# TF2-Engine/TF2

Hardware: AMD Instinct MI355X
Metric: images/sec ResNet50 INT4w/INT8a (higher is better)
Workload: dtype int8

## Files before the change

### tf2_amd/csrc/net.hip

```cpp
#include <hip/hip_runtime.h>
#include <algorithm>
#include <cstdio>
#include <cstdlib>
#include <cstring>
#include <map>
#include <mutex>
#include "tf2_net.h"
#include "tf2_device.h"
#include "opts.h"

namespace tf2 {

static thread_local std::string g_err;
void set_error(const std::string& s) { g_err = s; }
const std::string& last_error() { return g_err; }

#define HIP_OK(expr)                                                                   \
  do {                                                                                 \
    hipError_t e_ = (expr);                                                            \
    if (e_ != hipSuccess) {                                                            \
      set_error(std::string(#expr) + ": " + hipGetErrorString(e_));                    \
      return TF2_ERR_HIP;                                                              \
    }                                                                                  \
  } while (0)
// ... 280 lines not shown
  wp.scratch_bytes = (wp.scratch_bytes + 255) / 256 * 256;
  if (wp.ks_ctr_bytes) {
    wp.ks_part_off = wp.scratch_off + wp.scratch_bytes;
    wp.ks_part_bytes = (size_t)std::max(1, opts.sk_kb_blocks) * std::max(1, opts.sk_kb_max) * 16384;
    wp.scratch_bytes += wp.ks_part_bytes;
  }
  wp.total_bytes = wp.scratch_off + wp.scratch_bytes;
  auto res = plans.emplace(key, std::move(wp));
  return &res.first->second;
}

void Net::load_options() {
  RunOpts o;
  o.flags |= (int)opt("exp", 0) & 0x7ff8;
  o.pw_mode = (int)opt("pw", o.pw_mode);
  o.sk_mode = (int)opt("sk", o.sk_mode);
  o.sk8_blocks = (long)opt("sk8", o.sk8_blocks);
  o.bg_poll_limit = (long)opt("bgroup_polls", o.bg_poll_limit); o.bg_withhold = (long)opt("bgroup_withhold", 0);
  o.sk_s3_blocks = (long)opt("sk_s3", o.sk_s3_blocks); o.sk_s3_blocks_conc = (long)opt("sk_s3_conc", o.sk_s3_blocks_conc);
  o.fc_mode = (int)opt("fc", o.fc_mode);
  o.fc_min_slabs = (int)opt("fc_min", o.fc_min_slabs);
  o.c3_mode = (int)opt("c3", o.c3_mode);
  o.c3_min_blocks = (long)opt("c3_min", o.c3_min_blocks);
  o.c3_min256 = (long)opt("c3_min256", o.c3_min256);
  o.c3_w9 = (int)opt("c3_w9", o.c3_w9);
  o.c3_pool = (int)opt("c3_pool", o.c3_pool);
  o.first_fuse = (int)opt("first", o.first_fuse);
  o.first_pool = (int)opt("first_pool", o.first_pool);
  o.fire_mode = (int)opt("fire", o.fire_mode);
  o.fire_pool = (int)opt("fire_pool", o.fire_pool);
  o.bneck_min_blocks = (long)opt("bneck_min", o.bneck_min_blocks);
  o.stem_mode = (int)opt("stem", o.stem_mode);
  o.bgroup_min7 = (int)opt("bgroup_min7", o.bgroup_min7);
  o.bgroup_min14 = (int)opt("bgroup_min14", o.bgroup_min14);
  o.bgroup_min28 = (int)opt("bgroup_min28", o.bgroup_min28);
  o.bgroup_min56f = (int)opt("bgroup_min56f", o.bgroup_min56f);
  o.bgroup_chain = (int)opt("bgroup_chain", o.bgroup_chain);
  o.bgroup_mode = (int)opt("bgroup", o.bgroup_mode);
  o.bfirst_mode = (int)opt("bfirst", o.bfirst_mode);
  o.bfirst_min = (int)opt("bfirst_min", o.bfirst_min);
  o.bband_mode = (int)opt("bband", o.bband_mode);
  o.bband_rows = (int)opt("bband_rows", o.bband_rows);
  o.bband_rows_alone = (int)opt("bband_rows_alone", o.bband_rows_alone);
  o.bband_rows_dd = (int)opt("bband_rows_dd", o.bband_rows_dd);
  o.c3_min_hw = (int)opt("c3_min_hw", o.c3_min_hw);
  o.bband_min = (int)opt("bband_min", o.bband_min);
// ... 53 lines not shown
      if (st.sel == Launch::SEL_FIRST) { FirstArgs f = st.first; f.p = pa; return f.pool ? launch_conv_first_pool(f, stream) : launch_conv_first(f, stream); }
      return launch_prep_input(pa, stream);
    }
    case Launch::POOL: return launch_maxpool(st.pool, stream);
    case Launch::AVG: return launch_global_avg(st.avg, stream);
    case Launch::L2N: return launch_l2norm(st.l2n, stream);
    case Launch::CONV:
      switch (st.sel) {
        case Launch::SEL_PW: return launch_conv_pw(st.conv, st.TM, stream);
        case Launch::SEL_PWK: return launch_conv_pwk(st.conv, st.TM, stream);
        case Launch::SEL_PWKPAIR: return launch_conv_pwk_pair(st.conv, st.TM, st.conv2, st.TM2, stream);
        case Launch::SEL_SK:
          if (logits && lp->logits_direct >= 0 && &st == &lp->steps[lp->logits_direct]) {
            ConvArgs cd = st.conv_direct; cd.y = logits;
            return launch_conv_mfma_sk(cd, opts.sk8_blocks, st.shape, stream);
          }
          return launch_conv_mfma_sk(st.conv, opts.sk8_blocks, st.shape, stream);
        case Launch::SEL_MFMA2: return launch_conv_mfma2(st.conv, st.TM, stream);
        case Launch::SEL_BNECK: return launch_conv_bneck(st.bneck, st.TM, st.shape, stream);
        case Launch::SEL_PAIR: return launch_conv_mfma2_pair(st.conv, st.conv2, st.TM, stream);
        case Launch::SEL_SKPAIR: return launch_conv_mfma_sk_pair(st.conv, st.conv2, opts.sk8_blocks, st.shape, stream);
        case Launch::SEL_BBAND: return launch_conv_bband(st.bband, st.bg_c, st.bg_m, stream);
        case Launch::SEL_C3: return launch_conv_c3(st.c3, stream);
        case Launch::SEL_FIRE: return launch_conv_fire(st.fire, stream);
        case Launch::SEL_FC: return launch_conv_fc(st.fc, stream);
        case Launch::SEL_BGROUPF: return launch_conv_bgroup_first(st.bgroup, stream);
        case Launch::SEL_BFIRST: return launch_conv_bfirst(st.bgroup, stream);
        case Launch::SEL_BGROUP:
          if (!st.bg_chain.empty()) return launch_conv_bgroup(st.bg_chain.data(), (int)st.bg_chain.size(), st.bg_hw, st.bg_c, st.bg_m, stream);
          return launch_conv_bgroup(&st.bgroup, 1, st.bg_hw, st.bg_c, st.bg_m, stream);
        case Launch::SEL_STEM: return launch_conv_stem(st.stem, st.shape, stream);
        default: return launch_conv_shift(st.conv, st.signed_in, st.mul24, st.shape, stream);
      }
  }
  return -1;
}

tf2_status Net::describe_launches(int batch, bool concurrent, std::vector<std::pair<int, LaunchRecord>>* out) {
  std::lock_guard<std::mutex> lock(run_mutex);
  if (!packed_valid) { set_error("tf2_net_describe_launches: no packed image"); return TF2_ERR_STATE; }
  if (batch <= 0) { set_error("tf2_net_describe_launches: batch must be positive"); return TF2_ERR_ARG; }
  const WorkPlan* wp = plan(batch, false);
  const uint8_t* saved = packed_dev;
  if (!packed_dev) packed_dev = packed.data();
  static char fake_ws[16];
  std::list<LaunchPlan> keep;
// ... 246 lines not shown
```

### tf2_amd/csrc/net_plan.hip

```cpp
#include <hip/hip_runtime.h>
#include <algorithm>
#include <map>
#include <mutex>
#include <string>
#include <vector>
#include "tf2_net.h"
#include "tf2_device.h"

namespace tf2 {

bool Net::pair_candidate(int l) const {
  if (l < 1 || l + 1 >= nd.n_layers) return false;
  const tf2_layer_desc& A = layers[l]; const tf2_layer_desc& B = layers[l + 1];
  for (const tf2_layer_desc* L : {&A, &B})
    if (L->ipool || L->pool_en || L->endpool || L->concat >= 0 || L->src < 0) return false;
  if (B.src == l || B.add_src == l) return false;
  if (A.add_src >= 0 || B.add_src >= 0) return false;
  const PackLayer* pa = pack_layer(l); const PackLayer* pb = pack_layer(l + 1);
  if (!pa || !pb || pa->kind != KIND_MFMA || pb->kind != KIND_MFMA) return false;
  if (pa->fuse_next > 0 || pa->fused_into >= 0 || pb->fuse_next > 0 || pb->fused_into >= 0) return false;
  return true;
}

bool Net::bgroup_first_at(int l) const {
// ... 112 lines not shown
  if (L.ipool || L.k != 3 || L.stride != 1 || L.dil != 1 || L.pad_h != 1 || L.pad_w != 1 || L.src < 0 || L.add_src >= 0 || L.endpool) return false;
  if (layers[L.src].concat >= 0 || out_Cp[L.src] != L.C || L.OH != L.H || L.OW != L.W) return false;
  const PackLayer* pl = pack_layer(l);
  if (!pl || pl->kind != KIND_MFMA || (pl->TM != 64 && pl->TM != 128) || pl->w_share || pl->signed_in) return false;
  if (pl->Cp_in != L.C || pl->Cp_in % 64 != 0 || pl->nslab != 9 * (pl->Cp_in / 64) || (long)pl->n_entries != (long)pl->n_mtiles * pl->nslab) return false;
  if (pl->fuse_next > 0 || pl->fused_into >= 0) return false;
  const bool one_window = pl->n_phases == 1 && !pl->dual, dual = pl->n_phases == 2 && pl->dual;
  if (!one_window && !dual) return false;
  return conv_c3_shape_ok(L.H, L.W, L.C, pl->Np, opts.c3_min_hw);
}

bool Net::fc_at(int l, int batch) const {
  const tf2_layer_desc& L = layers[l];
  if (l == nd.n_layers - 1) return false;
  { const PackLayer* p4 = pack_layer(l); if (batch > 32 && !(p4 && p4->fc4)) return false; }
  if (L.ipool || L.k != L.H || L.k != L.W || L.stride != 1 || L.dil != 1 || L.pad_h || L.pad_w || L.OH != 1 || L.OW != 1) return false;
  if (L.src < 0 || L.add_src >= 0 || L.endpool || L.pool_en || L.concat >= 0 || layers[L.src].concat >= 0 || out_Cp[L.src] != L.C) return false;
  const PackLayer* pl = pack_layer(l);
  if (!pl || pl->kind != KIND_MFMA || (pl->TM != 64 && pl->TM != 128) || pl->w_share || pl->signed_in || pl->Np % 128 != 0) return false;
  if (pl->Cp_in != L.C || pl->Cp_in % 64 != 0 || pl->nslab != L.k * L.k * (pl->Cp_in / 64) || (long)pl->n_entries != (long)pl->n_mtiles * pl->nslab) return false;
  if ((pl->nslab < opts.fc_min_slabs && !pl->fc4) || pl->fuse_next > 0 || pl->fused_into >= 0) return false;
  const bool one_window = pl->n_phases == 1 && !pl->dual, dual = pl->n_phases == 2 && pl->dual;
  return one_window || dual;
}

bool Net::stem_selected(int batch) const {
  const tf2_layer_desc& L0 = layers[0];
  const PackLayer* p0 = pack_layer(0);
  const long long pixels = (long long)batch * L0.H * L0.W;
  return opts.stem_mode != 0 && p0 && p0->kind == KIND_MFMA && p0->off_w2 != 0 && nd.conv1_rewrite && nd.image_c == 3 &&
         in_layout[0].Cp_in == 64 && in_layout[0].half == 32 && L0.OH == L0.H - 2 && L0.OW == L0.W - 2 &&
         pixels * 64 < (1ll << 31) && (long long)batch * 3 * nd.image_h * nd.image_w < (1ll << 31);
}

static bool device_fits_group_launches() {
  int dev = 0;
  if (hipGetDevice(&dev) != hipSuccess) return true;
  static std::mutex mu;
  static std::map<int, int> n_cu;
  std::lock_guard<std::mutex> lock(mu);
  auto it = n_cu.find(dev);
  if (it == n_cu.end()) {
    hipDeviceProp_t prop;
    const int n = hipGetDeviceProperties(&prop, dev) == hipSuccess ? prop.multiProcessorCount : 256;
    it = n_cu.emplace(dev, n).first;
  }
// ... 385 lines not shown
    if (opts.c3_mode == 2) tmk = 64; else if (opts.c3_mode == 3 && pm->Np % 128 == 0) tmk = 128;
    Launch sc;
    if (!((long)batch * tiles * (pm->Np / tmk) >= opts.c3_min_blocks && conv_step(l, sc, false) && pm->TM == sc.TM)) return false;
    const ConvArgs& c = sc.conv;
    C3Args& f = sc.c3;
    f.x = c.x; f.y = c.y; f.w = c.w; f.hdr = c.hdr; f.hdr_bytes = c.hdr_bytes; f.zero2 = c.zero; f.tm = sc.TM; f.tmk = tmk;
    f.dbg = dbg_ptr(l);
    f.B = batch; f.H = L.H; f.W = L.W; f.C = L.C; f.M = pm->Np; f.x_cp = c.g.Cp_in;
    f.TH = th; f.TW = tw; f.tiles_x = tiles_x; f.tiles_per_img = tiles;
    set_fast_div((uint32_t)tw, &f.tw_m, &f.tw_s); set_fast_div((uint32_t)(tw + 2), &f.hc_m, &f.hc_s);
    set_fast_div((uint32_t)tiles_x, &f.tx_m, &f.tx_s); set_fast_div((uint32_t)tiles, &f.tpi_m, &f.tpi_s);
    f.relu = c.g.relu; f.fast = c.g.fast; f.dbl = c.g.dbl_out; f.dual = c.dual;
    f.y_cp = c.g.y_cp; f.y_off = c.g.y_off; f.y_nvalid = c.g.y_nvalid;
    if (pool_in) {
      const TensorPlan& to = T(E.out_tensor);
      f.pool = 1; f.PH = L.PH; f.PW = L.PW; f.y = base + to.offset; f.y_cp = to.Cp; f.y_off = E.out_off;
    }
    f.w9 = conv_c3_takes_w9(f, opts.c3_w9) ? 1 : 0;
    sc.sel = Launch::SEL_C3;
    st = sc;
    return pool_in;
  }

  bool bneck_fuse(int l, const tf2_layer_desc& L, const PackLayer* pl, Launch& st) {
    fused_done[pl->fuse_next] = 1;
    Launch sb;
    if (!conv_step(pl->fuse_next, sb, false)) return false;
    const PackLayer* pb = n.pack_layer(pl->fuse_next);
    BneckArgs& f = st.bneck;
    const ConvArgs& ca = st.conv; const ConvArgs& cb = sb.conv;
    f.x = ca.x; f.y_mid = ca.y; f.ymid_cp = ca.g.y_cp;
    f.w1 = ca.w; f.hdr1 = ca.hdr; f.hdr1_used = round_up((5 + pl->n_phases) * pl->TM * 4, 1024);
    f.dual1 = pl->dual; f.fast1 = pl->fast; f.relu1 = ca.g.relu;
    f.w2 = cb.w; f.hdr2 = cb.hdr; f.hdr2_bytes = cb.hdr_bytes; f.hdr2_used = round_up((5 + pb->n_phases) * pb->TM * 4, 1024);
    f.dual2 = pb->dual; f.fast2 = pb->fast; f.relu2 = cb.g.relu;
    f.y = cb.y; f.y_cp = cb.g.y_cp; f.y_off = cb.g.y_off; f.y_nvalid = cb.g.y_nvalid;
    f.res = cb.res; f.res_cp = cb.g.res_cp; f.res_off = cb.g.res_off; f.add_relu = cb.g.add_relu; f.has_res = cb.g.has_res;
    f.zero = ca.zero; f.keep_mid = wp->keep_all ? 1 : 0; f.dbl_mid = pl->off_dbl != 0; f.dbl_out = pb->off_dbl != 0;
    f.rnn = n.res_nonneg_single_clamp(pl->fuse_next) ? 1 : 0;
    f.B = batch; f.H = L.H; f.W = L.W; f.probe = opts.flags;
    f.dbg = dbg_ptr(l);
    set_fast_div((uint32_t)L.W, &f.w_m, &f.w_s); set_fast_div((uint32_t)(L.W + 2), &f.wp_m, &f.wp_s);
    const int TN = pl->TM == 64 ? 256 : 128;
    f.R = std::min(TN / L.W, L.H);
    f.tiles_per_img = (L.H + f.R - 1) / f.R;
    st.sel = Launch::SEL_BNECK; st.shape = TN;
// ... 86 lines not shown
    FirstArgs& f = s0.first;
    f.w = ca.w; f.hdr = ca.hdr; f.y = ca.y; f.im = s0.prep.y;
    f.hdr_used = hdr_used; f.dual = ca.dual; f.relu = ca.g.relu; f.fast = ca.g.fast; f.dbl = ca.g.dbl_out;
    f.y_cp = ca.g.y_cp; f.y_off = ca.g.y_off; f.y_nvalid = ca.g.y_nvalid; f.keep = wp->keep_all ? 1 : 0;
    f.pool = pooled ? 1 : 0;
    if (pooled) {
      const TensorPlan& to = T(E.out_tensor);
      f.yp = base + to.offset; f.PH = L.PH; f.PW = L.PW; f.ppad = L.pool_pad; f.yp_cp = to.Cp; f.yp_off = E.out_off;
    }
    s0.sel = Launch::SEL_FIRST; s0.layer = 0;
    return true;
  }

  void plain_row(int l) {
    const tf2_layer_desc L = n.exec_desc(l);
    const LayerExec& E = wp->exec[l];
    const PackLayer* pl = n.pack_layer(l);
    const bool fuse_now = bneck_fuses_now(L, pl);
    Launch st;
    if (!conv_step(l, st, !fuse_now)) { give_up(); return; }
    if (!fuse_now) fc_takeover(l, st);
    if (pl->fc4 && st.sel != Launch::SEL_FC) { give_up("layer " + std::to_string(l) + " is packed as 4-bit codes (fc4) but conv_fc cannot take it"); return; }
    const bool c3_pool_fused = !fuse_now && st.sel != Launch::SEL_FC && c3_takeover(l, L, st);
    if (fuse_now && !bneck_fuse(l, L, pl, st)) { give_up(); return; }
    if (opts.pair_mode && !fuse_now && !pair_forms(l, st)) { give_up(); return; }
    if (l == 0 && stem && !stem_step(L, pl, st)) { give_up(); return; }
    logits_direct(l, L, st);
    if (l == 0 && !fuse_now && first_fuse(L, pl, st)) return;
    lp.steps.push_back(st);
    const TensorPlan& tc = T(E.conv_tensor);
    if (L.pool_en && !(l == 0 && stem_pool_fused) && !(c3_pool_fused && st.sel == Launch::SEL_C3)) pool_step(l, tc, base + tc.offset, L.OH, L.OW);
    if (L.endpool && !st.avg_fused) avg_step(l, L);
  }

  bool rows() {
    for (int l = 0; l < nl && !failed; l++) {
      const PackLayer* pl = n.pack_layer(l);
      if (pl->merged_into >= 0) continue;
      if (n.layers[l].ipool == 2) { l2norm_step(l); continue; }
      if (n.layers[l].ipool) { const TensorPlan& ti = T(wp->exec[l].in_tensor); pool_step(l, ti, base + ti.offset, ti.H, ti.W); continue; }
      if (pl->fused_into >= 0 && fused_done[l]) continue;
      if (pair_done[l]) continue;
      if (try_bfirst(l) || try_group_first(l) || try_fire(l) || try_bband(l) || try_bgroup(l)) continue;
      plain_row(l);
    }
    return !failed;
// ... 56 lines not shown
```

### tf2_amd/csrc/opts.cpp

```cpp
#include <cstdio>
#include <cstdlib>
#include <cstring>
#include <cctype>
#include <unistd.h>
#include <map>
#include <memory>
#include <mutex>
#include "opts.h"

extern char** environ;

namespace tf2 {

namespace {
struct OptSpec { const char* name; int test_only; const char* doc; };
const OptSpec kOptSpecs[] = {
  {"alt_conc", 0, "how Net::run decides that batches are in flight: 0 never, 1 always, 2 (default) the caller's tf2_net_run_ex statement, else calls on >= 2 streams among the last eight"},
  {"bgroup", 0, "group launches (conv_bgroup.hip: eight co-resident blocks per image that meet inside the kernel) one batch at a time: 1 (default) / 0"},
  {"bfirst", 0, "the first bottleneck of the 56 x 56 stage (shortcut | reduce, 3x3, expand + residual) as one launch of independent row bands (conv_bfirst.hip): 0 never, 1 (default) with batches in flight, 2 one batch at a time as well"},
  {"bband", 0, "band launches (conv_bband.hip) of identity bottlenecks: 0 never, 1 (default) with batches in flight, 2 one batch at a time as well"},
  {"c3", 0, "3x3 / 1 / pad 1 layers of big maps on conv_c3.hip: 1 (default), 0 the ring kernel; 2 / 3 force 64- / 128-channel blocks (tests)"},
  {"fc", 0, "whole-window layers at batch <= 32 on conv_fc.hip (weight stream): 1 (default) / 0"},
  {"fc4", 0, "pack time: conv_fc layers keep their filters as 4-bit codes in HBM (expanded in registers): 1 (default) / 0 int8 window tiles"},
  {"share", 0, "pack time: alternative tile heights share the main entry's weight tiles: 1 (default: the wide ones), 2 all, 0 none"},
  {"merge", 1, "pack time: 0 = no merged rows (a 1x1 row and the 3x3 row behind it as one 3x3 layer)"},
  {"nodbl", 1, "pack time: no doubled channels"}, {"nofuse", 1, "pack time: no conv_bneck pairs"}, {"nodual", 1, "pack time: two-window layers in the Horner form"},
  {"nofast", 1, "pack time: generic requantisation everywhere"}, {"nosemi", 1, "pack time: no SEMI requantisation"}, {"nounit", 1, "pack time: conv1's low window as a window"},
  {"no4bit", 1, "pack time: shift-kernel layers keep int32 weights"}, {"im2col0", 1, "0: a 3x3 first layer on 3 channels keeps its plain form"},
  {"pw", 1, "conv_pw: 1 auto, 0 never"}, {"pw_slabs", 1, "conv_pw: most K slabs"}, {"pw_minpix", 1, "conv_pw: fewest pixels"},
  {"sk_kb", 1, "split-K launches of a few blocks split K over blocks as well (batch 1-4): 1 (default) / 0"}, {"sk_kb_blocks", 1, "... largest grid that takes it (default 8)"}, {"sk_kb_max", 1, "... most blocks per output tile (default 8)"}, {"sk_kb_min", 1, "... fewest (default 8: only slab lists long enough for eight parts)"}, {"stem_pk_small", 1, "conv_stem_pool_kernel at small batches: fewer pooled rows per block (>= ~192 blocks): 1 (default) / 0"}, {"q128", 1, "the input preparation reports -128s per image to conv_stem_pool_kernel (no scan of its input tile): 1 (default) / 0"}, {"pwk", 1, "conv_pwk (1x1 rows of 128 / 256 / 512 input channels: a block's weight fragments resident in registers, pixel tiles streamed through LDS): 0 never, 1 (default) with batches in flight, 2 one batch at a time as well"}, {"pwk_minpix", 1, "conv_pwk: fewest pixels"}, {"pwk_sk", 1, "conv_pwk: split-K rows as well"}, {"pwk_rows", 1, "bit mask of rows forced onto conv_pwk where the kernel can run them at all"}, {"nopwk_rows", 1, "... kept off it"}, {"pwk_slabs", 1, "conv_pwk: most K slabs of a row (2, 4 or 8)"}, {"pwk_units", 1, "conv_pwk: fewest (tile, channel part) units of a row (default 512)"}, {"pwk_pipe", 1, "conv_pwk: 0 = no requantisation between the next column group's MFMAs"}, {"pwk_slots", 1, "conv_pwk: blocks a launch aims at (0: 256, one per CU)"},
  {"sk", 1, "split-K kernel: 0 auto, 1 forced, 2 never"}, {"sk8", 1, "largest split-K grid in the 8-wave form"}, {"sk_s3", 1, "largest split-K grid on three ring stages, one batch at a time"}, {"sk_s3_conc", 1, "... with batches in flight"},
  {"fc_min", 1, "conv_fc: shortest K in slabs"}, {"c3_min", 1, "conv_c3: smallest grid"}, {"c3_min_hw", 1, "conv_c3: smallest map side (default 14)"}, {"c3_min256", 1, "conv_c3: smallest grid of 256-channel blocks"},
  {"fire", 1, "a fire module (squeeze + merged expands) as one launch: 0 never, 1 wherever it fits, 2 (default) on maps >= 28 wide"},
  {"fire_pool", 1, "fire modules with a pool behind their expands: 0 never, 1 / 2 fire launch + pool launch (maps >= 56 wide / wherever fire allows), 3 (default) the pool inside the fire launch one batch at a time, 4 always"},
  {"first", 1, "a 3x3 / stride 1 first layer on the image in one launch with its input preparation: 1 / 0"},
  {"first_pool", 1, "... a 3x3 first layer (stride 1 / 2) with a 3x3 / 2 max pool behind its ReLU, the pool included: 1 / 0"},
  {"c3_pool", 1, "a layer's 2x2 / 2 max pool inside its conv_c3 launch: 1 / 0"},
  {"c3_w9", 1, "conv_c3_w9_kernel: 0 never, 1 auto, 2 wherever allowed"},
  {"bneck_min", 1, "conv_bneck: smallest grid"}, {"stem", 1, "conv_stem: 1 auto, 0 never"}, {"stem_pool", 1, "conv1's pool in its launch"},
  {"avg_fuse", 1, "a layer's global average in its split-K launch: 0 never, 1 always, 2 (default) one batch at a time only"}, {"pair", 1, "pair launches"},
  {"bgroup_min7", 1, "smallest batch of the 7x7 group launches"}, {"bgroup_min14", 1, "... 14x14"}, {"bgroup_min28", 1, "... 28x28"}, {"bgroup_min56f", 1, "... the first 56x56 bottleneck"},
  {"bgroup_chain", 1, "identity bottlenecks per group launch"},
  {"bgroup_polls", 1, "group launches: polls of a meeting before it is reported as failed (default 1 << 24)"},
  {"bgroup_withhold", 1, "group launches: 1 + index of a block that leaves its group at kernel entry (the failure path of tf2_net_poll_error)"},
  {"bband_rows", 1, "band launches: rows per block with batches in flight"}, {"bband_rows_alone", 1, "... one batch at a time"},
  {"bband_rows_dd", 1, "band launches: most rows per block of a 28x28 bottleneck with two-window reduce and 3x3 (default 7; rounds 4-5: 4)"},
  {"bfirst_min", 1, "conv_bfirst: smallest batch"}, {"bband_min", 1, "band launches: smallest batch"}, {"bband_alone_maps", 1, "maps taking band launches one batch at a time (bit 1: 28x28, bit 2: 14x14)"},
  {"dense", 1, "arithmetic gather words"}, {"dense_max", 1, "longest slab list that takes them on multi-round grids"},
  {"alt_min", 1, "smallest grid taking a wide-tile alternative"}, {"alt_min_conc", 1, "... with batches in flight"}, {"alt_narrow", 1, "largest grid taking a narrow alternative"},
  {"alt_rows", 1, "bit mask of rows forced onto their alternative tile height"}, {"noalt_rows", 1, "... kept off it"},
  {"sk_rows", 1, "bit mask of 64-row-tile rows forced onto the in-block split-K kernel"}, {"nosk_rows", 1, "... kept off it"},
  {"exp", 1, "timing-probe bits (-DTF2_PROBES builds)"}, {"skip_layers", 1, "lo-hi: launches left out (-DTF2_PROBES builds)"},
  {"dbgptr", 1, "tools: device buffer for per-layer stamps"}, {"dbgptr2", 1, "tools: device buffer for per-block stamps"}, {"dbglayer", 1, "tools: the layer dbgptr2 records"},
};
// ... 83 lines not shown
```

### tf2_amd/csrc/tf2_internal.h

```cpp
#pragma once
#include <cstdint>
#include <cstddef>
#include <string>
#include <vector>
#include "../../include/tf2_amd.h"

namespace tf2 {

constexpr int kInflat = 15;
constexpr int kAlphaInflat = 20;
constexpr uint32_t kPackMagic = 0x32465441u;
constexpr uint32_t kPackVersion = 33;

inline int round_up(int x, int m) { return (x + m - 1) / m * m; }

enum ConvKind : int32_t { KIND_NONE = 0, KIND_MFMA = 1, KIND_SHIFT = 2, KIND_L2NORM = 3 };

struct PackLayer {
  int32_t kind;
  int32_t TM;
  int32_t n_mtiles;
  int32_t n_phases;
  int32_t nslab;
  int32_t Np;
// ... 118 lines not shown

struct C3Args {
  const int8_t* x; int8_t* y;
  const int8_t* w;
  const int32_t* hdr;
  const int8_t* zero2;
  long long* dbg;
  int32_t hdr_bytes, tm;
  int32_t tmk;
  int32_t B, H, W, C, M;
  int32_t x_cp;
  int32_t TH, TW, tiles_x, tiles_per_img;
  uint32_t tw_m, hc_m, tx_m, tpi_m; int32_t tw_s, hc_s, tx_s, tpi_s;
  int32_t relu, fast, dbl, dual;
  int32_t y_cp, y_off, y_nvalid;
  int32_t pool, PH, PW;
  int32_t w9;
};
bool conv_c3_takes_w9(const C3Args& a, int mode);
bool conv_c3_pick_tile(int H, int W, int* TH, int* TW);
bool conv_c3_pick_tile_pool(int H, int W, int* TH, int* TW);
bool conv_c3_shape_ok(int H, int W, int C, int Np, int min_hw);
int launch_conv_c3(const C3Args& a, void* stream);
#ifdef TF2_CHECK_DMA
void conv_bband_check_counts(unsigned long long out[2]);
void conv_c3_check_counts(unsigned long long out[2]);
#endif

struct BneckArgs {
  const int8_t* x;
  int8_t* y_mid;
  int8_t* y;
  const int8_t* res;
  const int8_t* w1;
  const int8_t* w2;
  const int32_t* hdr1;
  const int32_t* hdr2;
  const int8_t* zero;
  int32_t hdr1_used, hdr2_bytes, hdr2_used;
  int32_t B, H, W, R, tiles_per_img;
  int32_t dual1, fast1, relu1, dual2, fast2, relu2, add_relu, has_res, keep_mid;
  int32_t dbl_mid;
  int32_t dbl_out;
  int32_t rnn;
  int32_t probe;
  int32_t ymid_cp, y_cp, y_off, y_nvalid, res_cp, res_off;
// ... 225 lines not shown
```

### tf2_amd/csrc/tf2_net.h

```cpp
#pragma once
#include <cstring>
#include <list>
#include <map>
#include <memory>
#include <mutex>
#include <string>
#include <vector>
#include "tf2_internal.h"

namespace tf2 {

struct LaunchRecord;

struct TensorPlan {
  int H = 0, W = 0, C = 0, Cp = 0;
  size_t bytes = 0;
  size_t offset = 0;
  int last_use = -1;
  int first_use = -1;
};

struct LayerExec {
  int in_tensor = -1;
  int out_tensor = -1;
// ... 3 lines not shown
  int res_off = 0;
  int out_off = 0;
};

enum PlanMode { PLAN_ORDINARY = 0, PLAN_KEEP_ALL = 1, PLAN_OUTPUTS = 2 };

struct WorkPlan {
  int batch = 0;
  bool keep_all = false;
  bool outputs_kept = false;
  std::vector<TensorPlan> tensors;
  std::vector<LayerExec> exec;
  int input_tensor = -1;
  int final_tensor = -1;
  size_t scratch_off = 0, scratch_bytes = 0;
  size_t ctrl_off = 0, ctrl_bytes = 0;
  size_t ks_ctr_off = 0, ks_ctr_bytes = 0;
  size_t ks_part_off = 0, ks_part_bytes = 0;
  size_t total_bytes = 0;
};

struct Launch {
  enum Kind { PREP, CONV, POOL, AVG, L2N } kind = CONV;
  enum Sel { SEL_MFMA2, SEL_SK, SEL_PW, SEL_PWK, SEL_PWKPAIR, SEL_SHIFT, SEL_BNECK, SEL_STEM, SEL_PAIR, SEL_SKPAIR, SEL_BGROUP, SEL_BGROUPF, SEL_BFIRST, SEL_BBAND, SEL_C3, SEL_FC, SEL_FIRST, SEL_FIRE } sel = SEL_MFMA2;
  int layer = -1;
  int TM = 0, signed_in = 0, mul24 = 0, shape = 0;
  int TM2 = 0;
  int avg_fused = 0;
  ConvArgs conv{};
  ConvArgs conv2{};
  ConvArgs conv_direct{};
  BneckArgs bneck{};
  FcArgs fc{};
  C3Args c3{};
  BBandArgs bband{};
  BGroupArgs bgroup{};
  int bg_hw = 0, bg_c = 0, bg_m = 0;
  const BGroupArgs& bg_chain_last() const { return bg_chain.empty() ? bgroup : bg_chain.back(); }
  std::vector<BGroupArgs> bg_chain;
  StemArgs stem{};
  PoolArgs pool{};
  AvgArgs avg{};
  PrepArgs prep{};
  FireArgs fire{};
  FirstArgs first{};
  L2NormArgs l2n{};
};

struct LaunchPlan {
  int batch = 0;
  const WorkPlan* wp = nullptr;
  void* ws = nullptr;
  const uint8_t* packed_dev = nullptr;
  int concurrent = 0;
  int groups = 0;
  std::vector<Launch> steps;
  int logits_direct = -1;
// ... 7 lines not shown
  int pw_mode = 1, sk_mode = 0;
  long bneck_min_blocks = 200;
  int fire_mode = 2;
  int fire_pool = 3;
  int first_fuse = 1;
  int first_pool = 1;
  int c3_pool = 1;
  int c3_w9 = 1;
  int pw_slabs = 1; long pw_minpix = 8192;
  int stem_pk_small = 1;
  int sk_kb = 1;
  int sk_kb_blocks = 8;
  int sk_kb_max = 8;
  int sk_kb_min = 8;
  int q128_flags = 1;
  int pwk_mode = 1;
  long pwk_minpix = 4096;
  int pwk_max_slabs = 4;
  unsigned long long pwk_rows = 0, nopwk_rows = 0;
  int pwk_sk = 0;
  int c3_mode = 1;
  int c3_min_hw = 14;
  long c3_min_blocks = 96;
  int fc_mode = 1;
  int fc_min_slabs = 64;
  long c3_min256 = 200;
  long alt_min_blocks = 200;
  long alt_narrow_blocks = 64;
  long alt_min_blocks_conc = 90;
  unsigned long long alt_rows = 0, noalt_rows = 0, sk_rows = 0, nosk_rows = 0;
  int alt_conc_mode = 2;
  int dense_max_slabs = 17;
  int dense_mode = 1;
  int bgroup_mode = 1;
  int bgroup_chain = 5;
  int bgroup_min7 = 12, bgroup_min14 = 12, bgroup_min28 = 12, bgroup_min56f = 12;
  int bfirst_mode = 2;
  int bfirst_min = 12;
  int bband_mode = 1;
  int bband_rows_dd = 7;
  int bband_rows = 7, bband_rows_alone = 2;
  int bband_alone_maps = 0;
  int bband_min = 8;
  int pair_mode = 1;
  int avg_fuse = 2;
  int stem_pool = 1;
// ... 42 lines not shown
  tf2_status quantization(const char* text, size_t len, int8_t* q, size_t cap, int32_t* n_read) const;
  tf2_status load_model(const float* model, size_t n_floats);
  tf2_status load_model_4bit(const uint8_t* bytes, size_t n_bytes);
  tf2_status finish_model();
  tf2_status pack(int mode);
  bool stem_selected(int batch) const;
  const PackLayer* pack_layer(int l) const;
  const PackLayer* pack_layer_alt(int l) const;
  bool pair_candidate(int l) const;
  uint64_t tables_hash() const;
  const WorkPlan* plan(int batch, int mode);
  bool is_sink(int l) const;
  const LaunchPlan* launch_plan(int batch, const WorkPlan* wp, void* ws, bool concurrent, bool allow_groups);
  size_t workspace_size(int batch, bool keep_all);
  tf2_status describe_workspace(int batch, bool keep_all, std::vector<TensorPlan>* tensors, std::vector<LayerExec>* rows);
  bool bgroup_first_at(int l) const;
  bool bband_at(int l, int rows) const;
  tf2_layer_desc exec_desc(int l) const;
  bool out_nonneg(int l) const;
  bool res_nonneg_single_clamp(int l) const;
  bool fire_at(int l) const;
  bool c3_at(int l) const;
  bool fc_at(int l, int batch) const;
  bool bgroup_at(int l) const;
  long long stat_steps = 0, stat_group_steps = 0, stat_inflight_steps = 0, stat_small_mask_steps = 0;
  void* recent_streams[8] = {};
  int recent_pos = 0;
  void load_options();
  size_t logits_bytes(int batch) const;
  tf2_status poll_error(int batch, void* ws, size_t ws_bytes, void* stream);
  tf2_status run(const void* images, bool images_are_q, int batch, void* ws, size_t ws_bytes,
                 int8_t* logits, void* stream, int concurrency = -1, void* mark_event = nullptr, int mark_after_layer = -1,
                 bool outputs_kept = false);
  int issue(const Launch& st, const LaunchPlan* lp, const void* images, bool images_are_q, int8_t* logits, void* stream);
  tf2_status describe_launches(int batch, bool concurrent, std::vector<std::pair<int, struct LaunchRecord>>* out);
  tf2_status read_layer(int layer, int batch, const void* ws, int8_t* dst, size_t cap, void* stream);
  void drain_profile();
};

const std::string& last_error();

struct M4Tensor {
  int min_exp = 0, dtype = 0;
  size_t N = 0, C = 0, H = 0, W = 0, cnt = 0, words_per_row = 0;
  const uint8_t* payload = nullptr;
  int code(size_t i) const {
// ... 18 lines not shown
```

Measured before the change: 79760.

## Add whole-image LDS-resident conv kernel for 7x7x512 3x3 layers

Adds conv_img.hip, a kernel in which each block holds two whole 7x7 images (with halo) of the 512-channel input in LDS. The block's eight waves split the K entries (taps times 64-channel slabs) among themselves, and the partial sums are reduced through LDS before a requantise epilogue. The planner routes eligible stride-1 3x3 layers of ResNet-50's last stage to this kernel by default when batches are in flight and batch >= 8. The aim is to reuse the input tile across all nine taps and avoid the ring/split-K kernels' repeated loads on small maps, at the cost of a cross-wave LDS reduction and a fairly small grid.

```diff
diff --git a/tf2_amd/csrc/conv_img.hip b/tf2_amd/csrc/conv_img.hip
--- /dev/null
+++ b/tf2_amd/csrc/conv_img.hip
@@ -0,0 +1,235 @@
+#include <hip/hip_runtime.h>
+#include <type_traits>
+#include "tf2_internal.h"
+#include "tf2_device.h"
+#include "requant_epilogue.h"
+
+namespace tf2 {
+
+using i32x4 = int __attribute__((ext_vector_type(4)));
+using i32x16 = int __attribute__((ext_vector_type(16)));
+
+#define TF2_GLOBAL_PTR(p) ((const __attribute__((address_space(1))) void*)(p))
+#define TF2_LDS_PTR(p) ((__attribute__((address_space(3))) void*)(p))
+
+template <int T, int N, class F>
+__device__ __forceinline__ void img_static_for(F& fn) {
+  if constexpr (T < N) { fn(std::integral_constant<int, T>{}); img_static_for<T + 1, N>(fn); }
+}
+
+constexpr int kImgG = 2;
+constexpr int kImgWaves = 8;
+
+template <int HW, int C, int KS>
+struct ImgShape {
+  static constexpr int PAD = (KS - 1) / 2, HP = HW + 2 * PAD;
+  static constexpr int NPIX = HW * HW, NHALO = HP * HP;
+  static constexpr int NSL = C / 64, NE = KS * KS * NSL;
+  static constexpr int NT = (kImgG * NPIX + 31) / 32;
+  static constexpr int HGRP = (kImgG * NHALO + 15) / 16;
+  static constexpr int SLABB = HGRP * 1024;
+  static constexpr int TILE_BYTES = NSL * SLABB;
+  static constexpr int PART_BYTES = 64 * NT * 32 * 4;
+  static constexpr int PRM_OFF = TILE_BYTES > 4 * PART_BYTES ? TILE_BYTES : 4 * PART_BYTES;
+  static_assert(C % 64 == 0 && (KS == 1 || KS == 3), "instantiated forms");
+  static_assert(NE % kImgWaves == 0, "the entry list splits evenly over the waves (both window forms)");
+  static_assert(NT == 4, "eight waves finish eight 32 x 32 tiles: two row tiles x four column tiles");
+};
+
+template <int HW, int C, int KS, bool DUAL>
+__global__ __launch_bounds__(512) void conv_img_kernel(ImgArgs a) {
+  using S = ImgShape<HW, C, KS>;
+  constexpr int PAD = S::PAD, HP = S::HP, NPIX = S::NPIX, NHALO = S::NHALO, NSL = S::NSL, NE = S::NE, NT = S::NT, HGRP = S::HGRP, SLABB = S::SLABB;
+  constexpr int NW = DUAL ? 2 : 1;
+  constexpr int NI = NW * NE / kImgWaves;
+  static_assert(NE % NI == 0, "a wave's items lie in one window");
+  constexpr int A_BYTES = NW * 64 * 64;
+  extern __shared__ __attribute__((aligned(16))) int8_t lds[];
+
+  const int tid = threadIdx.x;
+  const int lane = tid & 63;
+  const int wave = __builtin_amdgcn_readfirstlane(tid >> 6);
+  const int half = lane >> 5;
+  int8_t* const tile = lds;
+  int* const prm = reinterpret_cast<int*>(lds + S::PRM_OFF);
+
+  const int bid = blockIdx.x;
+  const int grp = bid / a.n_mtiles, mt = bid - grp * a.n_mtiles;
+  const int img0 = grp * kImgG;
+  const int n_img = (a.B - img0) < kImgG ? (a.B - img0) : kImgG;
+  const int n_px = n_img * NPIX;
+
+  {
+    const int8_t* h = reinterpret_cast<const int8_t*>(a.hdr) + (size_t)mt * a.hdr_bytes + lane * 16;
+    for (int i = wave; i * 1024 < a.hdr_used; i += kImgWaves)
+      __builtin_amdgcn_global_load_lds(TF2_GLOBAL_PTR(h + i * 1024), TF2_LDS_PTR(reinterpret_cast<int8_t*>(prm) + i * 1024), 16, 0, 0);
+    const int chunk = (lane & 3) ^ ((lane >> 4) & 3);
+    for (int gi = wave; gi < HGRP * NSL; gi += kImgWaves) {
+      const int s = gi / HGRP, g = gi - s * HGRP;
+      const int hh = g * 16 + (lane >> 2);
+      const int hi = hh / NHALO, hq = hh - hi * NHALO;
+      const int hr = hq / HP, hc = hq - hr * HP;
+      const int row = hr - PAD, col = hc - PAD;
+      const bool ok = hi < n_img && (unsigned)row < (unsigned)HW && (unsigned)col < (unsigned)HW;
+      const int8_t* src = ok ? a.x + ((size_t)(img0 + hi) * NPIX + row * HW + col) * C + s * 64 + chunk * 16
+                             : a.zero + s * 64 + chunk * 16;
+      __builtin_amdgcn_global_load_lds(TF2_GLOBAL_PTR(src), TF2_LDS_PTR(tile + s * SLABB + g * 1024), 16, 0, 0);
+    }
+  }
+  int h0[NT];
+#pragma unroll
+  for (int j = 0; j < NT; j++) {
+    int p = j * 32 + (lane & 31);
+    if (p >= n_px) p = 0;
+    const int pi = p / NPIX, q = p - pi * NPIX;
+    const int r = q / HW;
+    h0[j] = pi * NHALO + r * HP + (q - r * HW);
+  }
+
+  const int v0 = wave * NI;
+  const int win = v0 / NE, e0 = v0 - win * NE;
+  struct Afr { i32x4 k[2][2]; };
+  const int8_t* const wbase = a.w + ((size_t)mt * NE + e0) * A_BYTES + win * (64 * 64) + (lane & 31) * 64 + half * 16;
+  auto load_a = [&](Afr& f, int i) __attribute__((always_inline)) {
+    const int8_t* p = wbase + (size_t)i * A_BYTES;
+#pragma unroll
+    for (int rt = 0; rt < 2; rt++) {
+      f.k[rt][0] = *reinterpret_cast<const i32x4*>(p + rt * 2048);
+      f.k[rt][1] = *reinterpret_cast<const i32x4*>(p + rt * 2048 + 32);
+    }
+  };
+  Afr f0, f1, f2;
+  load_a(f0, 0);
+  if (NI > 1) load_a(f1, 1);
+
+  i32x16 acc[2][NT];
+#pragma unroll
+  for (int rt = 0; rt < 2; rt++)
+#pragma unroll
+    for (int j = 0; j < NT; j++)
+#pragma unroll
+      for (int r = 0; r < 16; r++) acc[rt][j][r] = 0;
+
+  asm volatile("s_waitcnt vmcnt(0)" ::: "memory");
+  __builtin_amdgcn_s_barrier();
+  asm volatile("" ::: "memory");
+
+  auto step = [&](auto i_c) __attribute__((always_inline)) {
+    constexpr int i = decltype(i_c)::value;
+    Afr& cur = i % 3 == 0 ? f0 : i % 3 == 1 ? f1 : f2;
+    Afr& nxt = (i + 2) % 3 == 0 ? f0 : (i + 2) % 3 == 1 ? f1 : f2;
+    if (i + 2 < NI) load_a(nxt, i + 2);
+    const int e = e0 + i;
+    const int t = e / NSL, s = e - t * NSL;
+    const int th = t / KS, toff = th * HP + (t - th * KS);
+    const int8_t* B = tile + s * SLABB;
+    int ba[NT];
+#pragma unroll
+    for (int j = 0; j < NT; j++) {
+      const int hh = h0[j] + toff;
+      ba[j] = hh * 64 + ((half ^ ((hh >> 2) & 3)) << 4);
+    }
+#pragma unroll
+    for (int ks = 0; ks < 2; ks++) {
+      i32x4 bf[NT];
+#pragma unroll
+      for (int j = 0; j < NT; j++) bf[j] = *reinterpret_cast<const i32x4*>(B + (ba[j] ^ (ks << 5)));
+#pragma unroll
+      for (int j = 0; j < NT; j++) {
+        acc[0][j] = __builtin_amdgcn_mfma_i32_32x32x32_i8(cur.k[0][ks], bf[j], acc[0][j], 0, 0, 0);
+        acc[1][j] = __builtin_amdgcn_mfma_i32_32x32x32_i8(cur.k[1][ks], bf[j], acc[1][j], 0, 0, 0);
+      }
+    }
+    __builtin_amdgcn_sched_barrier(0);
+  };
+  img_static_for<0, NI>(step);
+
+  auto part = [&](int slot, int rt, int j, int q) __attribute__((always_inline)) {
+    return reinterpret_cast<i32x4*>(lds + slot * S::PART_BYTES + ((rt * NT + j) * 4 + q) * 1024 + lane * 16);
+  };
+  auto store_acc = [&](int slot) __attribute__((always_inline)) {
+#pragma unroll
+    for (int rt = 0; rt < 2; rt++)
+#pragma unroll
+      for (int j = 0; j < NT; j++)
+#pragma unroll
+        for (int q = 0; q < 4; q++)
+          *part(slot, rt, j, q) = i32x4{acc[rt][j][4 * q], acc[rt][j][4 * q + 1], acc[rt][j][4 * q + 2], acc[rt][j][4 * q + 3]};
+  };
+  asm volatile("s_waitcnt lgkmcnt(0)" ::: "memory");
+  __builtin_amdgcn_s_barrier();
+  asm volatile("" ::: "memory");
+  if (wave >= 4) store_acc(wave - 4);
+  asm volatile("s_waitcnt lgkmcnt(0)" ::: "memory");
+  __builtin_amdgcn_s_barrier();
+  asm volatile("" ::: "memory");
+  if (wave < 4) {
+#pragma unroll
+    for (int rt = 0; rt < 2; rt++)
+#pragma unroll
+      for (int q = 0; q < 4; q++) {
+        i32x4 d = {0, 0, 0, 0};
+        if (DUAL) d = *reinterpret_cast<const i32x4*>(prm + (kPrmWordsPerRow + 1) * 64 + rt * 32 + 4 * half + 8 * q);
+#pragma unroll
+        for (int j = 0; j < NT; j++) {
+          const i32x4 o = *part(wave, rt, j, q);
+#pragma unroll
+          for (int r = 0; r < 4; r++)
+            acc[rt][j][4 * q + r] = (int)(((unsigned)acc[rt][j][4 * q + r] << (d[r] & 31)) + (unsigned)o[r]);
+        }
+      }
+    store_acc(wave);
+  }
+  asm volatile("s_waitcnt lgkmcnt(0)" ::: "memory");
+  __builtin_amdgcn_s_barrier();
+  asm volatile("" ::: "memory");
+
+  const int rt = wave >> 2, ct = wave & 3;
+  if (ct * 32 >= n_px) return;
+  int a16[16];
+#pragma unroll
+  for (int q = 0; q < 4; q++) {
+    i32x4 sum = *part(0, rt, ct, q);
+#pragma unroll
+    for (int sl = 1; sl < 4; sl++) {
+      const i32x4 o = *part(sl, rt, ct, q);
+#pragma unroll
+      for (int r = 0; r < 4; r++) sum[r] = (int)((unsigned)sum[r] + (unsigned)o[r]);
+    }
+#pragma unroll
+    for (int r = 0; r < 4; r++) a16[4 * q + r] = sum[r];
+  }
+  const int lo_bound = a.relu ? 0 : -128;
+  const i32x4 nores = {0, 0, 0, 0};
+  const i32x4 out = a.fast == 1 ? requant_tile16<false, 0, true>(a16, prm, 64, rt * 32 + 4 * half, lo_bound, -128, nores, a.dbl != 0)
+                                : requant_tile16<false, 0, false>(a16, prm, 64, rt * 32 + 4 * half, lo_bound, -128, nores, a.dbl != 0, a.fast == 2);
+  const int p = ct * 32 + (lane & 31);
+  const int ch = mt * 64 + rt * 32 + 16 * half;
+  if (p < n_px && ch + 16 <= a.y_nvalid)
+    *reinterpret_cast<i32x4*>(a.y + ((size_t)img0 * NPIX + p) * a.y_cp + a.y_off + ch) = out;
+}
+
+bool conv_img_shape_ok(int HW, int C, int k) { return HW == 7 && C == 512 && k == 3; }
+
+size_t conv_img_lds_bytes(int HW, int C, int k, size_t hdr_used) {
+  if (!conv_img_shape_ok(HW, C, k)) return 0;
+  return (size_t)ImgShape<7, 512, 3>::PRM_OFF + hdr_used;
+}
+
+long conv_img_blocks(int batch, int n_mtiles) { return (long)((batch + kImgG - 1) / kImgG) * n_mtiles; }
+
+int launch_conv_img(const ImgArgs& a, void* stream) {
+  hipStream_t s = (hipStream_t)stream;
+  if (!conv_img_shape_ok(a.HW, a.C, a.k) || a.hdr_used > a.hdr_bytes) return 1;
+  const size_t lds = conv_img_lds_bytes(a.HW, a.C, a.k, (size_t)a.hdr_used);
+  if (lds > 160 * 1024) return 1;
+  const long grid = conv_img_blocks(a.B, a.n_mtiles);
+#define TF2_IMG(D) do { auto fn = conv_img_kernel<7, 512, 3, D>; if (!lds_attr_once(reinterpret_cast<const void*>(fn))) return -1; \
+                        TF2_LAUNCH_NAME("conv_img_kernel<%dx%d,C%d,k%d,%s,%d images>", a.HW, a.HW, a.C, a.k, D ? "two-window" : "one-window", kImgG); \
+                        TF2_LAUNCH(fn, dim3((unsigned)grid), dim3(512), lds, s, a); } while (0)
+  if (a.dual) TF2_IMG(true); else TF2_IMG(false);
+#undef TF2_IMG
+  return launch_ok() ? 0 : -1;
+}
+
+}
diff --git a/tf2_amd/csrc/net.hip b/tf2_amd/csrc/net.hip
--- a/tf2_amd/csrc/net.hip
+++ b/tf2_amd/csrc/net.hip
@@ -326,6 +326,9 @@
   o.fc_min_slabs = (int)opt("fc_min", o.fc_min_slabs);
   o.c3_mode = (int)opt("c3", o.c3_mode);
   o.c3_min_blocks = (long)opt("c3_min", o.c3_min_blocks);
+  o.img_mode = (int)opt("img", o.img_mode);
+  o.img_min = (int)opt("img_min", o.img_min);
+  o.img_rows = (unsigned long long)opt("img_rows", 0); o.noimg_rows = (unsigned long long)opt("noimg_rows", 0);
   o.c3_min256 = (long)opt("c3_min256", o.c3_min256);
   o.c3_w9 = (int)opt("c3_w9", o.c3_w9);
   o.c3_pool = (int)opt("c3_pool", o.c3_pool);
@@ -425,6 +428,7 @@
         case Launch::SEL_SKPAIR: return launch_conv_mfma_sk_pair(st.conv, st.conv2, opts.sk8_blocks, st.shape, stream);
         case Launch::SEL_BBAND: return launch_conv_bband(st.bband, st.bg_c, st.bg_m, stream);
         case Launch::SEL_C3: return launch_conv_c3(st.c3, stream);
+        case Launch::SEL_IMG: return launch_conv_img(st.img, stream);
         case Launch::SEL_FIRE: return launch_conv_fire(st.fire, stream);
         case Launch::SEL_FC: return launch_conv_fc(st.fc, stream);
         case Launch::SEL_BGROUPF: return launch_conv_bgroup_first(st.bgroup, stream);
diff --git a/tf2_amd/csrc/net_plan.hip b/tf2_amd/csrc/net_plan.hip
--- a/tf2_amd/csrc/net_plan.hip
+++ b/tf2_amd/csrc/net_plan.hip
@@ -158,6 +158,22 @@
   if ((pl->nslab < opts.fc_min_slabs && !pl->fc4) || pl->fuse_next > 0 || pl->fused_into >= 0) return false;
   const bool one_window = pl->n_phases == 1 && !pl->dual, dual = pl->n_phases == 2 && pl->dual;
   return one_window || dual;
+}
+
+bool Net::img_at(int l) const {
+  if (l < 0 || l >= nd.n_layers - 1) return false;
+  const tf2_layer_desc& L = layers[l];
+  if (L.ipool || L.pool_en || L.endpool || L.concat >= 0 || L.add_src >= 0 || L.src < 0) return false;
+  if ((L.k != 1 && L.k != 3) || L.stride != 1 || L.dil != 1 || L.pad_h != (L.k - 1) / 2 || L.pad_w != (L.k - 1) / 2) return false;
+  if (L.H != L.W || L.OH != L.H || L.OW != L.W) return false;
+  if (layers[L.src].concat >= 0 || out_Cp[L.src] != L.C || !out_nonneg(L.src)) return false;
+  const PackLayer* pl = pack_layer(l);
+  if (!pl || pl->kind != KIND_MFMA || pl->TM != 64 || pl->w_share || pl->signed_in) return false;
+  if (pl->Cp_in != L.C || pl->Cp_in % 64 != 0 || pl->nslab != L.k * L.k * (pl->Cp_in / 64) || (long)pl->n_entries != (long)pl->n_mtiles * pl->nslab) return false;
+  if (pl->fuse_next > 0 || pl->fused_into >= 0 || pl->merge_next > 0 || pl->merged_into >= 0 || pl->fc4) return false;
+  const bool one_window = pl->n_phases == 1 && !pl->dual, dual = pl->n_phases == 2 && pl->dual;
+  if (!one_window && !dual) return false;
+  return conv_img_shape_ok(L.H, L.C, L.k);
 }
 
 bool Net::stem_selected(int batch) const {
@@ -589,6 +605,27 @@
     return pool_in;
   }
 
+  void img_takeover(int l, const tf2_layer_desc& L, Launch& st) {
+    if (l < 64 && ((opts.noimg_rows >> l) & 1)) return;
+    const bool forced = l < 64 && ((opts.img_rows >> l) & 1);
+    if (!(forced || (opts.img_mode && (concurrent || opts.img_mode == 2) && batch >= opts.img_min))) return;
+    if (!n.img_at(l)) return;
+    const PackLayer* pm = n.pack_layer(l);
+    Launch sc;
+    if (!(conv_step(l, sc, false) && sc.TM == 64 && pm->TM == 64)) return;
+    const ConvArgs& c = sc.conv;
+    if ((long long)batch * L.H * L.W * std::max(c.g.Cp_in, c.g.y_cp) >= (1ll << 32) || c.g.Cp_in != L.C || c.g.has_res || c.g.avg_mult) return;
+    ImgArgs& f = sc.img;
+    f.x = c.x; f.y = c.y; f.w = c.w; f.hdr = c.hdr; f.hdr_bytes = c.hdr_bytes; f.zero = c.zero;
+    f.hdr_used = round_up((5 + pm->n_phases) * 64 * 4, 1024);
+    f.B = batch; f.HW = L.H; f.C = L.C; f.k = L.k; f.n_mtiles = pm->n_mtiles;
+    f.dual = c.dual; f.relu = c.g.relu; f.fast = c.g.fast; f.dbl = c.g.dbl_out;
+    f.y_cp = c.g.y_cp; f.y_off = c.g.y_off; f.y_nvalid = c.g.y_nvalid;
+    if (f.hdr_used > f.hdr_bytes || conv_img_lds_bytes(f.HW, f.C, f.k, (size_t)f.hdr_used) > 160 * 1024) return;
+    sc.sel = Launch::SEL_IMG; sc.avg_fused = 0;
+    st = sc;
+  }
+
   bool bneck_fuse(int l, const tf2_layer_desc& L, const PackLayer* pl, Launch& st) {
     fused_done[pl->fuse_next] = 1;
     Launch sb;
@@ -721,6 +758,7 @@
     if (!fuse_now) fc_takeover(l, st);
     if (pl->fc4 && st.sel != Launch::SEL_FC) { give_up("layer " + std::to_string(l) + " is packed as 4-bit codes (fc4) but conv_fc cannot take it"); return; }
     const bool c3_pool_fused = !fuse_now && st.sel != Launch::SEL_FC && c3_takeover(l, L, st);
+    if (!fuse_now && st.sel != Launch::SEL_FC && st.sel != Launch::SEL_C3 && !st.avg_fused) img_takeover(l, L, st);
     if (fuse_now && !bneck_fuse(l, L, pl, st)) { give_up(); return; }
     if (opts.pair_mode && !fuse_now && !pair_forms(l, st)) { give_up(); return; }
     if (l == 0 && stem && !stem_step(L, pl, st)) { give_up(); return; }
diff --git a/tf2_amd/csrc/opts.cpp b/tf2_amd/csrc/opts.cpp
--- a/tf2_amd/csrc/opts.cpp
+++ b/tf2_amd/csrc/opts.cpp
@@ -20,6 +20,7 @@
   {"bfirst", 0, "the first bottleneck of the 56 x 56 stage (shortcut | reduce, 3x3, expand + residual) as one launch of independent row bands (conv_bfirst.hip): 0 never, 1 (default) with batches in flight, 2 one batch at a time as well"},
   {"bband", 0, "band launches (conv_bband.hip) of identity bottlenecks: 0 never, 1 (default) with batches in flight, 2 one batch at a time as well"},
   {"c3", 0, "3x3 / 1 / pad 1 layers of big maps on conv_c3.hip: 1 (default), 0 the ring kernel; 2 / 3 force 64- / 128-channel blocks (tests)"},
+  {"img", 0, "stride-1 rows of small square maps (ResNet-50's 7 x 7 x 512 3x3 rows) on conv_img.hip (whole images per block, the input resident in LDS): 0 never, 1 (default) with batches in flight, 2 one batch at a time as well (group launches keep their rows)"},
   {"fc", 0, "whole-window layers at batch <= 32 on conv_fc.hip (weight stream): 1 (default) / 0"},
   {"fc4", 0, "pack time: conv_fc layers keep their filters as 4-bit codes in HBM (expanded in registers): 1 (default) / 0 int8 window tiles"},
   {"share", 0, "pack time: alternative tile heights share the main entry's weight tiles: 1 (default: the wide ones), 2 all, 0 none"},
@@ -30,6 +31,7 @@
   {"pw", 1, "conv_pw: 1 auto, 0 never"}, {"pw_slabs", 1, "conv_pw: most K slabs"}, {"pw_minpix", 1, "conv_pw: fewest pixels"},
   {"sk_kb", 1, "split-K launches of a few blocks split K over blocks as well (batch 1-4): 1 (default) / 0"}, {"sk_kb_blocks", 1, "... largest grid that takes it (default 8)"}, {"sk_kb_max", 1, "... most blocks per output tile (default 8)"}, {"sk_kb_min", 1, "... fewest (default 8: only slab lists long enough for eight parts)"}, {"stem_pk_small", 1, "conv_stem_pool_kernel at small batches: fewer pooled rows per block (>= ~192 blocks): 1 (default) / 0"}, {"q128", 1, "the input preparation reports -128s per image to conv_stem_pool_kernel (no scan of its input tile): 1 (default) / 0"}, {"pwk", 1, "conv_pwk (1x1 rows of 128 / 256 / 512 input channels: a block's weight fragments resident in registers, pixel tiles streamed through LDS): 0 never, 1 (default) with batches in flight, 2 one batch at a time as well"}, {"pwk_minpix", 1, "conv_pwk: fewest pixels"}, {"pwk_sk", 1, "conv_pwk: split-K rows as well"}, {"pwk_rows", 1, "bit mask of rows forced onto conv_pwk where the kernel can run them at all"}, {"nopwk_rows", 1, "... kept off it"}, {"pwk_slabs", 1, "conv_pwk: most K slabs of a row (2, 4 or 8)"}, {"pwk_units", 1, "conv_pwk: fewest (tile, channel part) units of a row (default 512)"}, {"pwk_pipe", 1, "conv_pwk: 0 = no requantisation between the next column group's MFMAs"}, {"pwk_slots", 1, "conv_pwk: blocks a launch aims at (0: 256, one per CU)"},
   {"sk", 1, "split-K kernel: 0 auto, 1 forced, 2 never"}, {"sk8", 1, "largest split-K grid in the 8-wave form"}, {"sk_s3", 1, "largest split-K grid on three ring stages, one batch at a time"}, {"sk_s3_conc", 1, "... with batches in flight"},
+  {"img_min", 1, "conv_img: smallest batch (default 8)"}, {"img_rows", 1, "bit mask of rows taken by conv_img whatever img / img_min say, where the kernel can run them at all"}, {"noimg_rows", 1, "... kept off it"},
   {"fc_min", 1, "conv_fc: shortest K in slabs"}, {"c3_min", 1, "conv_c3: smallest grid"}, {"c3_min_hw", 1, "conv_c3: smallest map side (default 14)"}, {"c3_min256", 1, "conv_c3: smallest grid of 256-channel blocks"},
   {"fire", 1, "a fire module (squeeze + merged expands) as one launch: 0 never, 1 wherever it fits, 2 (default) on maps >= 28 wide"},
   {"fire_pool", 1, "fire modules with a pool behind their expands: 0 never, 1 / 2 fire launch + pool launch (maps >= 56 wide / wherever fire allows), 3 (default) the pool inside the fire launch one batch at a time, 4 always"},
diff --git a/tf2_amd/csrc/tf2_internal.h b/tf2_amd/csrc/tf2_internal.h
--- a/tf2_amd/csrc/tf2_internal.h
+++ b/tf2_amd/csrc/tf2_internal.h
@@ -164,6 +164,21 @@
 bool conv_c3_pick_tile_pool(int H, int W, int* TH, int* TW);
 bool conv_c3_shape_ok(int H, int W, int C, int Np, int min_hw);
 int launch_conv_c3(const C3Args& a, void* stream);
+
+struct ImgArgs {
+  const int8_t* x; int8_t* y;
+  const int8_t* w;
+  const int32_t* hdr;
+  const int8_t* zero;
+  int32_t hdr_bytes, hdr_used;
+  int32_t B, HW, C, k, n_mtiles;
+  int32_t dual, relu, fast, dbl;
+  int32_t y_cp, y_off, y_nvalid;
+};
+bool conv_img_shape_ok(int HW, int C, int k);
+size_t conv_img_lds_bytes(int HW, int C, int k, size_t hdr_used);
+long conv_img_blocks(int batch, int n_mtiles);
+int launch_conv_img(const ImgArgs& a, void* stream);
 #ifdef TF2_CHECK_DMA
 void conv_bband_check_counts(unsigned long long out[2]);
 void conv_c3_check_counts(unsigned long long out[2]);
diff --git a/tf2_amd/csrc/tf2_net.h b/tf2_amd/csrc/tf2_net.h
--- a/tf2_amd/csrc/tf2_net.h
+++ b/tf2_amd/csrc/tf2_net.h
@@ -49,7 +49,7 @@
 
 struct Launch {
   enum Kind { PREP, CONV, POOL, AVG, L2N } kind = CONV;
-  enum Sel { SEL_MFMA2, SEL_SK, SEL_PW, SEL_PWK, SEL_PWKPAIR, SEL_SHIFT, SEL_BNECK, SEL_STEM, SEL_PAIR, SEL_SKPAIR, SEL_BGROUP, SEL_BGROUPF, SEL_BFIRST, SEL_BBAND, SEL_C3, SEL_FC, SEL_FIRST, SEL_FIRE } sel = SEL_MFMA2;
+  enum Sel { SEL_MFMA2, SEL_SK, SEL_PW, SEL_PWK, SEL_PWKPAIR, SEL_SHIFT, SEL_BNECK, SEL_STEM, SEL_PAIR, SEL_SKPAIR, SEL_BGROUP, SEL_BGROUPF, SEL_BFIRST, SEL_BBAND, SEL_C3, SEL_FC, SEL_FIRST, SEL_FIRE, SEL_IMG } sel = SEL_MFMA2;
   int layer = -1;
   int TM = 0, signed_in = 0, mul24 = 0, shape = 0;
   int TM2 = 0;
@@ -60,6 +60,7 @@
   BneckArgs bneck{};
   FcArgs fc{};
   C3Args c3{};
+  ImgArgs img{};
   BBandArgs bband{};
   BGroupArgs bgroup{};
   int bg_hw = 0, bg_c = 0, bg_m = 0;
@@ -113,6 +114,9 @@
   int c3_mode = 1;
   int c3_min_hw = 14;
   long c3_min_blocks = 96;
+  int img_mode = 1;
+  int img_min = 8;
+  unsigned long long img_rows = 0, noimg_rows = 0;
   int fc_mode = 1;
   int fc_min_slabs = 64;
   long c3_min256 = 200;
@@ -201,6 +205,7 @@
   bool fire_at(int l) const;
   bool c3_at(int l) const;
   bool fc_at(int l, int batch) const;
+  bool img_at(int l) const;
   bool bgroup_at(int l) const;
   long long stat_steps = 0, stat_group_steps = 0, stat_inflight_steps = 0, stat_small_mask_steps = 0;
   void* recent_streams[8] = {};
```

After: 80690 (median of 6 runs). +1.2%, better.
